# USNavalResearchLaboratory/mgen

Hardware: AMD Instinct MI355X
Metric: device-resident MgenMsg pack+unpack GB/s and Mmsg/s at 1/2/4/8 MI355X (higher is better)
Workload: dtype u8; 1 GPU; udp_unpack_crc_1M_x_1024B; records_per_gpu=1048576, record_bytes=1024, checksum=True, output=mgenx_rec rows (32 B), parallelism=flow-sharded x1 (independent slabs)

## Files before the change

### mgen_amd/csrc/mgenx_api.hip

```cpp
#include <hipcub/hipcub.hpp>
#include <hsa/hsa.h>
#include <hsa/hsa_ext_amd.h>
#include <immintrin.h>

#include <math.h>
#include <stdio.h>
#include <string.h>

#include <algorithm>
#include <chrono>
#include <emmintrin.h>
#include <atomic>
#include <mutex>
#include <vector>


#include "mgenx_kernels.hpp"
#include "mgenx_flowdist.hpp"
#if MGENX_DIAG
#include "mgenx_diag.h"
#endif

extern "C" void* mgenx_scan_ws_new();
extern "C" void mgenx_scan_ws_free(void* p);
// ... 353 lines not shown
  for (mgenx_worker* w : c->workers) worker_detach(w);
  c->workers.clear();
  void* ps[] = {c->d_tabs, c->d_expect, c->d_xpow, c->d_ia, c->d_bytetab, c->d_rtab, c->d_rcrc,
                c->d_sink, c->d_rq};
  if (c->scan_ws) mgenx_scan_ws_free(c->scan_ws);
  if (c->flow_ws) mgenx_flow_ws_free(c->flow_ws);
  if (c->flowdist_ws) mgenx_flowdist_ws_free(c->flowdist_ws);
  if (c->log_ws) mgenx_log_ws_free(c->log_ws);
  mgenx::dev_free(c->tcp_ws);
  mgenx::dev_free(c->tcp_plan);
  mgenx::dev_free(c->rx_ws);
  mgenx::host_free(c->tcp_host);
  for (mgenx_grow& g : c->bl) g.release();
  c->snap.release();
  c->defrag.release();
  c->lp.release();
  for (void* p : ps) mgenx::dev_free(p);
  delete c;
  return MGENX_OK;
}

int mgenx_unpack_batch(mgenx_ctx* ctx, const uint8_t* dev_slab, uint64_t slab_bytes,
                       const uint64_t* dev_rec_off, uint64_t stride,
                       const uint32_t* dev_rec_len, uint32_t fixed_len, uint32_t n,
                       const mgenx_cols* cols, uint32_t opts, void* stream) {
  if (!ctx || !cols) return MGENX_EINVAL;
  if (n == 0) return MGENX_OK;
  if (!dev_slab) return MGENX_EINVAL;
  if (!dev_rec_off && stride == 0 && n > 1) return MGENX_EINVAL;
  const mgenx_cols& k = *cols;
  if (!k.rows && (!k.flow_id || !k.seq_num || !k.tx_sec || !k.tx_usec || !k.msg_len ||
                  !k.dst_port || !k.flags || !k.err || !k.dst_type || !k.dst_len ||
                  !k.dst_addr4 || !k.payload_len || !k.payload_type || !k.gps_status))
    return MGENX_EINVAL;
  mgenx::UnpackParams p;
  p.slab = dev_slab;
  p.slab_bytes = slab_bytes;
  p.rec_off = dev_rec_off;
  p.stride = stride;
  p.rec_len = dev_rec_len;
  p.fixed_len = fixed_len;
  p.n = n;
  p.opts = opts;
  p.tabs = ctx->d_tabs;
  p.expect = ctx->d_expect;
  p.expect_fixed = fixed_len < ctx->h_expect.size() ? ctx->h_expect[fixed_len] : 0u;
  p.sink = ctx->d_sink;
  p.variant = MGENX_DIAG ? ctx->unpack_variant : 0;
  p.cols = k;
  const uint64_t groups = ((uint64_t)n + 15) / 16;
  const uint64_t per_block = (uint64_t)mgenx::unpack_threads() / 64;
  uint64_t grid = (groups + per_block - 1) / per_block;
  if (grid > (uint64_t)ctx->cu_count) grid = ctx->cu_count;
  hipError_t e = mgenx::launch_unpack(p, (int)grid, (hipStream_t)stream, &ctx->unpack_last);
  return e == hipSuccess ? MGENX_OK : set_err(ctx, e, "unpack");
}

int mgenx_unpack_last_kernel(const mgenx_ctx* ctx) { return ctx ? ctx->unpack_last : 0; }

int mgenx_pack_prepare(mgenx_ctx* ctx, const mgenx_flow_tmpl* dev_tmpl, uint32_t n_tmpl,
                       const uint8_t* dev_pool, uint32_t* dev_tmpl_crc, void* stream) {
  if (!ctx || (n_tmpl && (!dev_tmpl || !dev_tmpl_crc))) return MGENX_EINVAL;
  hipError_t e = mgenx::launch_pack_prepare(dev_tmpl, n_tmpl, dev_pool, ctx->d_bytetab,
                                            dev_tmpl_crc, (hipStream_t)stream);
  return e == hipSuccess ? MGENX_OK : set_err(ctx, e, "pack_prepare");
}

int mgenx_set_fill_time(mgenx_ctx* ctx, uint32_t fill_time) {
  if (!ctx) return MGENX_EINVAL;
  if (ctx->rand_ready && ctx->rand_time == fill_time) return MGENX_OK;
  std::vector<uint8_t> rt(16 + kN + 32, 0);
  glibc_rand_bytes(fill_time, kN, &rt[16]);
  uint32_t t[256];
  byte_table(t);
  std::vector<uint32_t> rc(kN);
  uint32_t c = 0;
  for (uint32_t k = 0; k < kN; k++) {
    rc[k] = c;
    c = t[(c ^ rt[16 + k]) & 0xffu] ^ (c >> 8);
  }
  hipSetDevice(ctx->device);
  hipError_t e = hipMemcpy(ctx->d_rtab, rt.data(), rt.size(), hipMemcpyHostToDevice);
  if (e == hipSuccess) e = hipMemcpy(ctx->d_rcrc, rc.data(), kN * 4, hipMemcpyHostToDevice);
  if (e != hipSuccess) return set_err(ctx, e, "set_fill_time");
  ctx->rand_ready = true;
  ctx->rand_time = fill_time;
  return MGENX_OK;
}

static int pack_common(mgenx_ctx* ctx, const mgenx_flow_tmpl* dev_tmpl,
                       const uint32_t* dev_tmpl_crc, const mgenx_pack_desc* dev_desc, uint32_t n,
                       const uint8_t* dev_pool, uint8_t* dev_slab, uint64_t slab_bytes,
                       const uint64_t* dev_rec_off, uint64_t stride, const uint32_t* dev_buf_len,
                       const uint32_t* dev_crc_in, uint32_t* dev_out_len, uint32_t* dev_tx_crc,
                       uint32_t* dev_state, uint32_t opts, uint32_t fill_time, void* stream,
                       const uint32_t* dev_frag_len = nullptr, int frag_ck = 0,
                       const uint32_t* dev_skip = nullptr) {
  if (!ctx) return MGENX_EINVAL;
  if (n == 0) return MGENX_OK;
  if (!dev_tmpl || !dev_tmpl_crc || !dev_desc || !dev_slab || !dev_out_len) return MGENX_EINVAL;
  if (!dev_rec_off && stride == 0 && n > 1) return MGENX_EINVAL;
  if (opts & MGENX_PACK_RANDOM_FILL) {
    if (!ctx->rand_ready || ctx->rand_time != fill_time) return MGENX_EINVAL;
  }
  mgenx::PackParams p;
  p.tmpl = dev_tmpl;
  p.tmpl_crc = dev_tmpl_crc;
// ... 1296 lines not shown
```

### mgen_amd/csrc/mgenx_kernels.hpp

```cpp
#pragma once

#include "mgenx_common.hpp"

#include <mutex>
#include <set>
#include <utility>

#ifndef MGENX_DIAG
#define MGENX_DIAG 0
#endif

namespace mgenx {

void quiesce_workers(int device);
inline void dev_free(void* p) {
  if (!p) return;
  int dev = -1;
  if (hipGetDevice(&dev) != hipSuccess) dev = -1;
  quiesce_workers(dev);
  (void)hipFree(p);
}
inline void host_free(void* p) {
  if (!p) return;
  quiesce_workers(-1);
// ... 8 lines not shown
  static std::set<std::pair<const void*, int>> done;
  std::lock_guard<std::mutex> g(mu);
  if (done.count({fn, dev})) return hipSuccess;
  e = hipFuncSetAttribute(fn, hipFuncAttributeMaxDynamicSharedMemorySize, bytes);
  if (e == hipSuccess) done.insert({fn, dev});
  return e;
}

struct UnpackParams {
  const uint8_t* slab;
  uint64_t slab_bytes;
  const uint64_t* rec_off;
  uint64_t stride;
  const uint32_t* rec_len;
  uint32_t fixed_len;
  uint32_t n;
  uint32_t opts;
  const uint32_t* tabs;
  const uint32_t* expect;
  uint32_t expect_fixed;
  uint8_t* sink;
  int variant;
  mgenx_cols cols;
};

struct PackParams {
  const mgenx_flow_tmpl* tmpl;
  const uint32_t* tmpl_crc;
  const mgenx_pack_desc* desc;
  uint32_t n;
  const uint8_t* pool;
  uint8_t* slab;
  uint64_t slab_bytes;
  const uint64_t* rec_off;
  uint64_t stride;
  uint32_t* out_len;
  uint32_t opts;
  const uint32_t* byte_tab;
  const uint32_t* a4_tab;
  const uint32_t* xpow;
  const uint32_t* ia;
  const uint8_t* rtab;
  const uint32_t* rcrc;
  const uint32_t* buf_len;
  const uint32_t* crc_in;
  uint32_t* tx_crc;
  uint32_t* state;
  const uint32_t* frag_len;
  int frag_ck;
  int variant;
  const uint32_t* skip = nullptr;
};

hipError_t launch_unpack(const UnpackParams& p, int grid, hipStream_t stream, int* which);
int unpack_threads();
#if MGENX_DIAG
hipError_t launch_group_rw(const uint8_t* p, uint64_t bytes, uint8_t* out, int mode, int grid,
                           hipStream_t stream);
hipError_t launch_stream_read(const uint8_t* p, uint64_t bytes, uint32_t* out, int grid,
                              hipStream_t stream);
hipError_t launch_stream_read_w(const uint8_t* p, uint64_t bytes, uint32_t* out, int grid,
                                int width, hipStream_t stream);
#endif
hipError_t launch_pack(const PackParams& p, int grid, hipStream_t stream);
hipError_t launch_pack_prepare(const mgenx_flow_tmpl* tmpl, uint32_t n_tmpl, const uint8_t* pool,
                               const uint32_t* byte_tab, uint32_t* out, hipStream_t stream);
constexpr int kRqUnqTime = 0;
constexpr int kRqThrTime = 256;
constexpr int kRqLog10Lo = -40;
constexpr int kRqLog10N = 65;
constexpr int kRqThrLog10 = 512;
constexpr int kRqP10 = 512 + 65;
constexpr int kRqP10N = 309;
constexpr int kRqDoubles = 512 + 65 + 309;

hipError_t launch_rx_persist(const mgenx_cols& c, uint32_t n, uint32_t opts, int32_t* ws,
                             mgenx_rx_state* state, const uint8_t* slab, const uint64_t* rec_off,
                             const uint32_t* rec_len, const uint32_t* byte_tab,
                             uint32_t* payload_rec, hipStream_t s);
size_t rx_persist_ws_bytes(uint32_t n);
hipError_t launch_tcp_plan(const mgenx_flow_tmpl* tmpl, const mgenx_pack_desc* desc,
                           const uint32_t* msg_total, uint32_t n, uint64_t* bytes,
                           uint32_t* nfrag, uint32_t* max_frag, hipStream_t s);
hipError_t launch_tcp_frag(const mgenx_pack_desc* desc, const uint32_t* msg_total,
                           const uint32_t* nfrag, const uint64_t* msg_off, uint32_t n, uint32_t r,
                           int ck, const uint32_t* prev_state, mgenx_pack_desc* fd, uint64_t* foff,
                           uint32_t* fbuf, uint32_t* ff, hipStream_t s);
constexpr uint32_t kTcpPlanMsgs = 1024;
constexpr uint32_t kTcpPlanEpochs = 1u << 16;
hipError_t launch_tcp_plan0(const mgenx_flow_tmpl* tmpl, const mgenx_pack_desc* desc,
                            const uint32_t* msg_total, uint32_t n, int ck, uint64_t cap,
                            uint32_t epoch, uint64_t* status, uint64_t* fmax, uint64_t* msg_off,
                            uint32_t* nfrag, mgenx_pack_desc* fd, uint32_t* fbuf, uint32_t* ff,
                            uint32_t* skip, uint64_t* host, hipStream_t s);
constexpr uint32_t kWorkUnpack = 1, kWorkCrc32 = 2, kWorkPack = 3, kWorkRecv = 4, kWorkUpdate = 5,
                   kWorkStop = 15;
constexpr uint32_t kWorkerMaxBytes = MGENX_WORKER_MAX_BYTES;
constexpr uint32_t kWorkerHdrBytes = 1024;
constexpr uint32_t kWorkerPackMax = MGENX_WORKER_PACK_MAX;
struct WPackReq {
  mgenx_flow_tmpl tmpl;
  mgenx_pack_desc desc;
  uint32_t buf_len, crc_in, opts, rsv;
};
struct WUpdReq {
  uint64_t flows;
  uint32_t slot, seq, rx_sec, rx_usec, tx_sec, tx_usec, msg, rsv;
// ... 30 lines not shown
```

### mgen_amd/csrc/mgenx_unpack.hip

```cpp
#include <type_traits>

#include "mgenx_kernels.hpp"
#include "mgenx_parse.hpp"

namespace mgenx {

constexpr int kUnpackThreads = 1024;
constexpr int kRep = 32;
constexpr int kRepDwords = 4 * 256 * kRep;
constexpr int kSmallTabDwords = 1024;
constexpr int kFoldTabs = 6;
constexpr size_t kUnpackLdsBytes = (size_t)(kRepDwords + kFoldTabs * kSmallTabDwords) * 4u;


__device__ __forceinline__ uint32_t a64_s1(uint32_t lane) { return ((lane & 31u) << 2) | (1u << 16); }

typedef __attribute__((address_space(3))) uint32_t lds_u32_t;
__device__ __forceinline__ uint32_t lds_u32(const uint8_t*, uint32_t addr, uint32_t imm) {
  return *(const lds_u32_t*)(addr + imm);
}

__device__ __forceinline__ uint32_t xor3(uint32_t a, uint32_t b, uint32_t c) {
  return __builtin_amdgcn_bitop3_b32(a, b, c, 0x96);
}

__device__ __forceinline__ void a64_parts(const uint8_t* ldsb, uint32_t c, uint32_t s1,
                                          uint32_t& ha, uint32_t& hb) {
  const uint32_t t0 = lds_u32(ldsb, __builtin_amdgcn_perm(c, s1, 0x0c0c0400u), 0);
  const uint32_t t1 = lds_u32(ldsb, __builtin_amdgcn_perm(c, s1, 0x0c0c0500u), 128);
  const uint32_t t2 = lds_u32(ldsb, __builtin_amdgcn_perm(c, s1, 0x0c020600u), 0);
  const uint32_t t3 = lds_u32(ldsb, __builtin_amdgcn_perm(c, s1, 0x0c020700u), 128);
  ha = xor3(t0, t1, t2);
  hb = t3;
}

struct TableRegs {
  uint32_t a64, fold[kFoldTabs];
};
__device__ __forceinline__ TableRegs table_loads(const uint32_t* tabs) {
  TableRegs r;
  r.a64 = tabs[threadIdx.x];
#pragma unroll
  for (int k = 0; k < kFoldTabs; k++) r.fold[k] = tabs[1024 + k * 1024 + threadIdx.x];
  return r;
}
__device__ __forceinline__ void table_writes(uint32_t* lds, const TableRegs& r) {
  typedef __attribute__((address_space(3))) u32x4_t lds_u32x4_t;
  const uint32_t e = threadIdx.x;
  const uint32_t k = e >> 8, val = e & 255u;
  const u32x4_t s = {r.a64, r.a64, r.a64, r.a64};
  lds_u32x4_t* dst = (lds_u32x4_t*)((k >> 1) * 65536u + val * 256u + (k & 1u) * 128u);
#pragma unroll
  for (int c = 0; c < kRep / 4; c++) dst[c] = s;
  uint32_t* fold = lds + kRepDwords;
#pragma unroll
  for (int k2 = 0; k2 < kFoldTabs; k2++) fold[k2 * 1024 + e] = r.fold[k2];
}
__device__ __forceinline__ void stage_tables(uint32_t* lds, const uint32_t* tabs) {
  table_writes(lds, table_loads(tabs));
}

__device__ __forceinline__ uint32_t shift_tab(const uint32_t* t, uint32_t x) {
  return t[x & 0xffu] ^ t[256 + ((x >> 8) & 0xffu)] ^ t[512 + ((x >> 16) & 0xffu)] ^
         t[768 + (x >> 24)];
}

__device__ __forceinline__ u32x4_t shl_bytes(u32x4_t v, int s) {
  const int a = s >> 2;
  const int c = (s & 3) * 8;
  uint32_t w[4] = {v.x, v.y, v.z, v.w};
  uint32_t o[4];
#pragma unroll
  for (int i = 0; i < 4; i++) {
    const int hi_i = i - a, lo_i = i - a - 1;
    uint32_t hi = 0, lo = 0;
#pragma unroll
    for (int k = 0; k < 4; k++) {
      hi = (k == hi_i) ? w[k] : hi;
      lo = (k == lo_i) ? w[k] : lo;
    }
    o[i] = c ? ((hi << c) | (lo >> (32 - c))) : hi;
  }
  return u32x4_t{o[0], o[1], o[2], o[3]};
}


__device__ __forceinline__ bool fast_layout(uint32_t w0, uint32_t w5, uint32_t hw) {
  const uint32_t t = (w5 >> 16) & 0xffu;
  const uint32_t D = w5 >> 24;
  const uint32_t H = hw >> 24;
  return ((w0 >> 16) & 0xffu) == 2u && (t == 1u || t == 2u) && (D == 4u || D == 16u) &&
         (H == 0u || H == 4u || H == 16u) && D + H <= 20u;
}

__device__ bool small_crc_ok(const uint8_t* r, uint32_t L) {
  if (L < 4) return false;
  uint32_t c = 0xFFFFFFFFu;
  for (uint32_t i = 0; i < L - 4; i++) {
    c ^= r[i];
#pragma unroll
    for (int k = 0; k < 8; k++) c = (c >> 1) ^ ((c & 1u) ? kPoly : 0u);
  }
  c ^= 0xFFFFFFFFu;
  const uint32_t t = ((uint32_t)r[L - 4] << 24) | ((uint32_t)r[L - 3] << 16) |
                     ((uint32_t)r[L - 2] << 8) | r[L - 1];
  return c == t;
}

__device__ __forceinline__ uint32_t prefix_word(const u32x4_t& pf, int k) {
// ... 773 lines not shown
        } else {
#pragma unroll
          for (int j = 0; j < 8; j++) w[j] = 0;
        }
        const bool flagged = force || (((w[0] >> 24) & MGENX_FLAG_CHECKSUM) != 0 &&
                                       buf_len >= MGENX_MIN_SIZE && ((w[0] >> 16) & 0xffu) == 2u);
        const bool needs_crc = flagged && (tcp ? (G.L >= 4) : fixed_ok(buf_len, w));
        const bool vec_crc = needs_crc && G.L >= 32;
        Hdr h;
        parse_header(rec, buf_len, want_ext, w, h);
        const bool crc_ok = !needs_crc || (vec_crc ? (tot == expect) : small_crc_ok(rec, G.L));
        store_hdr_q0(p.cols, G.idx, h, crc_ok, tcp);
      } else if (G.oob && q == 0) {
        store_oob_q0(p.cols, G.idx);
      }
    }

    if (KB > 0 && burst && held == (uint32_t)KH) flush();
    if (!has_next) break;
    pf = ldu128(hdr_ptr(N));
    expect = p.expect[N.live ? N.L : 0u];
    if (next_tile) {
      t_c = t_p;
      t_p = t_c + n_waves;
      off_c = off_p;
      len_c = len_p;
      src_c = src_p;
      place(t_p, off_p, len_p);
      p_ranked = false;
      k = 0;
    } else {
      k++;
    }
    G = N;
  }
  if (KB > 0 && burst && held) flush();
}

template <int NR, int MODE = 0, bool kRows = false, bool kAligned = false>
__global__ void __launch_bounds__(kUnpackThreads)
unpack_fixed_kernel(UnpackParams p, uint32_t expect) {
  constexpr bool kAblXor = (MODE & 1) != 0, kAblNoTail = (MODE & 2) != 0;
  constexpr bool kAblNoStore = (MODE & 4) != 0, kAblSink = (MODE & 8) != 0;
  constexpr bool kAblAltStore = (MODE & 16) != 0;
  constexpr bool kAblWrap = (MODE & 32) != 0;
  constexpr bool kAblWt = (MODE & 64) != 0;
  constexpr bool kAblNtLoad = (MODE & 128) != 0;
  constexpr bool kAblBurst = (MODE & 256) != 0;
  constexpr bool kAblBurstSeq = (MODE & 512) != 0;
  extern __shared__ __attribute__((aligned(16))) uint32_t lds[];
  uint32_t* rep = lds;
  uint32_t* fold = lds + kRepDwords;
  const uint8_t* ldsb = reinterpret_cast<const uint8_t*>(rep);
  const TableRegs tab_regs = table_loads(p.tabs);
  asm volatile("" ::: "memory");

  const int lane = threadIdx.x & 63;
  const int q = lane & 3;
  const uint32_t s1 = a64_s1((uint32_t)lane);
  const uint32_t wave_id = __builtin_amdgcn_readfirstlane(
      blockIdx.x * (blockDim.x >> 6) + (threadIdx.x >> 6));
  const uint32_t n_waves = gridDim.x * (blockDim.x >> 6);
  const uint32_t n_groups = (p.n + 15u) >> 4;
  const bool force = (p.opts & MGENX_OPT_CHECKSUM_FORCE) != 0;
  const bool tcp = (p.opts & MGENX_OPT_TCP) != 0;
  const uint32_t L = p.fixed_len;
  constexpr int V = NR;

  uint32_t g = wave_id;
  const uint32_t g_end = n_groups;

  auto rec_idx = [&](uint32_t gg) { return (gg << 4) + (uint32_t)(lane >> 2); };
  auto rec_ptr = [&](uint32_t i) { return p.slab + (uint64_t)i * p.stride; };
  auto is_live = [&](uint32_t i) {
    const uint64_t off = (uint64_t)i * p.stride;
    return i < p.n && off <= p.slab_bytes && L <= p.slab_bytes - off;
  };
  auto base_off = [&](bool lv, uint32_t i) { return lv ? i * (uint32_t)p.stride : 64u; };
  const int pos0 = (int)L - 64 * V + 16 * q;
  auto ld = [&](uint32_t off, int imm) {
    if (kAblNtLoad) return ldnt128(p.slab + (uint64_t)off + imm);
    return ldu128(p.slab + (uint64_t)off + imm);
  };
  auto ld_row = [&](uint32_t boff, int j) {
    return j == 0 ? ld(boff + (uint32_t)(pos0 > 0 ? pos0 : 0), 0)
                  : ld(boff + (uint32_t)(pos0 + 64), 64 * (j - 1));
  };
  auto ld_hdr = [&](uint32_t boff) { return ld(boff + 16u * (uint32_t)q, 0); };

  u32x4_t d[NR];
  struct Out {
    uint32_t o[5];
  };
  auto decode = [&](const u32x4_t& pf, uint32_t idx, bool live) {
    uint32_t w[8];
#pragma unroll
    for (int j = 0; j < 8; j++) w[j] = prefix_word(pf, j);
    const uint32_t w10 = prefix_word(pf, 10);
    const uint32_t D = w[5] >> 24;
    const uint32_t hw = (D == 4u) ? w[7] : w10;
    const uint32_t gi = (28u + D + (hw >> 24)) >> 2;
    const uint32_t g3 = (prefix_word(pf, 11) & (0u - (uint32_t)(gi == 8u))) |
                        (prefix_word(pf, 12) & (0u - (uint32_t)(gi == 9u))) |
                        (prefix_word(pf, 14) & (0u - (uint32_t)(gi == 11u))) |
                        (prefix_word(pf, 15) & (0u - (uint32_t)(gi == 12u)));
    uint32_t flow = bswap32(w[1]), seq = bswap32(w[2]), sec = bswap32(w[3]);
    uint32_t usec = bswap32(w[4]), dst4 = w[6];
// ... 190 lines not shown
      __builtin_amdgcn_sched_barrier(0);
      const uint32_t v = shift_tab(fold + 3 * 1024, f0) ^ shift_tab(fold + 2 * 1024, f1) ^
                         shift_tab(fold + 1 * 1024, f2) ^ shift_tab(fold, f3);
      const uint32_t* lt = fold + (q == 0 ? 5 : (q == 1 ? 4 : 3)) * 1024;
      uint32_t s = (q == 3) ? v : shift_tab(lt, v);
      s ^= __shfl_xor(s, 1);
      s ^= __shfl_xor(s, 2);
      if (kAblNoTail) {
        if (s == 0x9E3779B9u && lane == 0) p.cols.err[idx] = (uint8_t)needs_crc;
      } else {
        const Out r = kAligned ? early : decode(hdr, idx, live);
        emit(r, idx, needs_crc && s != expect);
      }
      asm volatile("" ::"v"(boff_n + (uint32_t)(pos0 + 64)));
      g = gn;
      idx = idx_n;
      live = live_n;
      return has_next && any;
    };
    u32x4_t pf2;
    if (kAligned) {
      while (step(pf, pf2)) {
      }
    } else {
      for (;;) {
        if (!step(pf, pf2)) break;
        if (!step(pf2, pf)) break;
      }
    }
    for (; g < g_end; g += n_waves) {
      const uint32_t i = rec_idx(g);
      const bool lv = is_live(i);
      const u32x4_t ph = ld_hdr(base_off(lv, i));
      const bool nc = decide(ph, lv);
      if (__any(nc)) break;
      emit(decode(ph, i, lv), i, false);
    }
  }
  if (kAblBurst) {
    uint32_t k = 0;
    for (uint32_t gg = wave_id; gg < g_end; gg += n_waves, k++) {
      const uint32_t i = rec_idx(gg);
      const uint64_t seq = (uint64_t)wave_id * 8192u + k * 512u + 8u * (uint32_t)lane;
      const uint64_t a = (uint64_t)p.cols.rows + (kAblBurstSeq ? seq : (uint64_t)i * 32 + 8 * q);
      if (i < p.n) {
        if (kAblWt) st_g64_wt(a, (uint64_t)gg);
        else if (kAblAltStore) st_g64(a, (uint64_t)gg);
        else st_g64_nt(a, (uint64_t)gg);
      }
    }
  }
}

template <int NR, int RS = 4, int K = 16>
__global__ void __launch_bounds__(kUnpackThreads)
unpack_fixed_ring_kernel(UnpackParams p, uint32_t expect) {
  static_assert(NR == 8 || NR == 16, "ring kernel: 512- or 1024-byte records");
  static_assert(NR % RS == 0, "the ring divides the record's rows");
  extern __shared__ __attribute__((aligned(16))) uint32_t lds[];
  const uint32_t* fold = lds + kRepDwords;
  const uint8_t* ldsb = reinterpret_cast<const uint8_t*>(lds);
  const TableRegs tab_regs = table_loads(p.tabs);
  asm volatile("" ::: "memory");

  const int lane = threadIdx.x & 63;
  const int q = lane & 3;
  const uint32_t s1 = a64_s1((uint32_t)lane);
  const uint32_t wave_id = __builtin_amdgcn_readfirstlane(
      blockIdx.x * (blockDim.x >> 6) + (threadIdx.x >> 6));
  const uint32_t n_waves = gridDim.x * (blockDim.x >> 6);
  const uint32_t g_end = (p.n + 15u) >> 4;
  const bool force = (p.opts & MGENX_OPT_CHECKSUM_FORCE) != 0;
  const bool tcp = (p.opts & MGENX_OPT_TCP) != 0;
  const uint32_t L = p.fixed_len;

  auto rec_idx = [&](uint32_t gg) { return (gg << 4) + (uint32_t)(lane >> 2); };
  auto is_live = [&](uint32_t i) {
    const uint64_t off = (uint64_t)i * p.stride;
    return (bool)((i < p.n) & (off <= p.slab_bytes) & (L <= p.slab_bytes - off));
  };
  auto row_base = [&](uint32_t i, bool live) {
    return (live ? i * (uint32_t)p.stride : 64u) + 16u * (uint32_t)q;
  };
  const uint32_t qm0 = 0u - (uint32_t)(q == 0), qm1 = 0u - (uint32_t)(q == 1);
  const uint32_t qm2 = 0u - (uint32_t)(q == 2), qm3 = 0u - (uint32_t)(q == 3);
  auto ld = [&](uint32_t base, int j) { return ldu128(p.slab + (uint64_t)base + 64 * j); };
  auto decide = [&](const u32x4_t& pf, bool live) {
    const uint32_t w0 = prefix_word(pf, 0);
    const uint32_t w5 = prefix_word(pf, 5);
    const bool v2 = ((w0 >> 16) & 0xffu) == 2u;
    const bool flagged = force || ((((w0 >> 24) & MGENX_FLAG_CHECKSUM) != 0) && v2);
    const uint32_t t = (w5 >> 16) & 0xffu;
    return live && flagged && (tcp || (v2 && (t == 1u || t == 2u)));
  };
  auto decode = [&](const u32x4_t& pf, uint32_t idx, bool live, uint32_t& o0, uint32_t& o1) {
    uint32_t w[8];
#pragma unroll
    for (int j = 0; j < 8; j++) w[j] = prefix_word(pf, j);
    const uint32_t w10 = prefix_word(pf, 10);
    const uint32_t D = w[5] >> 24;
    const uint32_t hw = (D == 4u) ? w[7] : w10;
    const uint32_t gi = (28u + D + (hw >> 24)) >> 2;
    const uint32_t g3 = (prefix_word(pf, 11) & (0u - (uint32_t)(gi == 8u))) |
                        (prefix_word(pf, 12) & (0u - (uint32_t)(gi == 9u))) |
                        (prefix_word(pf, 14) & (0u - (uint32_t)(gi == 11u))) |
                        (prefix_word(pf, 15) & (0u - (uint32_t)(gi == 12u)));
    uint32_t flow = bswap32(w[1]), seq = bswap32(w[2]), sec = bswap32(w[3]);
    uint32_t usec = bswap32(w[4]), dst4 = w[6];
    uint32_t msg_len = bswap16((uint16_t)(w[0] & 0xffffu));
    uint32_t dport = bswap16((uint16_t)(w[5] & 0xffffu));
    const uint32_t hlen = 44u + D + (hw >> 24);
    uint32_t plen = bswap16((uint16_t)(g3 >> 16));
    if (!(plen != 0 && hlen + plen <= L)) plen = 0;
    uint32_t flags = w[0] >> 24, err = 0, dtype = (w[5] >> 16) & 0xffu, dlen = D;
    uint32_t ptype = (g3 >> 8) & 0xffu, gps = g3 & 0xffu;
    const bool slow = live && !fast_layout(w[0], w[5], hw);
    if (__any(slow)) {
      Hdr h;
      if (slow && q == 0) parse_header(p.slab + (uint64_t)idx * p.stride, L, false, w, h);
      auto bc = [&](uint32_t& dst, uint32_t v) {
        v = (uint32_t)__builtin_amdgcn_mov_dpp((int)v, 0x00, 0xf, 0xf, false);
        if (slow) dst = v;
      };
      bc(flow, h.flow); bc(seq, h.seq); bc(sec, h.sec); bc(usec, h.usec); bc(dst4, h.dst4);
      bc(msg_len, h.msg_len); bc(dport, h.dst_port); bc(plen, h.plen); bc(flags, h.flags);
      bc(err, h.err); bc(dtype, h.dst_type); bc(dlen, h.dst_len); bc(ptype, h.ptype);
      bc(gps, h.gps);
    }
    const uint32_t a3 = plen | flags << 16 | err << 24;
    const uint32_t c3 = dtype | dlen << 8 | ptype << 16 | gps << 24;
    const uint32_t c2 = msg_len | dport << 16;
    const uint32_t r0 = (flow & qm0) | (sec & qm1) | (dst4 & qm2) | (a3 & qm3);
    const uint32_t r1 = (seq & qm0) | (usec & qm1) | (c2 & qm2) | (c3 & qm3);
    o0 = live ? r0 : (qm3 & ((uint32_t)MGENX_ERROR_OOB << 24));
    o1 = live ? r1 : 0u;
  };
  auto verdict = [&](uint32_t& o0, bool crc_bad) {
    const uint32_t fl = tcp ? (uint32_t)MGENX_FLAG_CHECKSUM_ERROR : 0u;
    if (crc_bad && q == 3) o0 = (o0 & 0x00ffffffu) | fl << 16 | (uint32_t)MGENX_ERROR_CHECKSUM << 24;
  };

  typedef uint32_t held_t __attribute__((ext_vector_type(K)));
  held_t b0 = 0u, b1 = 0u;
  uint32_t held = 0, last_g = 0;
  uint32_t left = __builtin_amdgcn_readfirstlane(
      wave_id < g_end ? (g_end - 1u - wave_id) / n_waves + 1u : 0u);
  uint32_t slot = (uint32_t)K - (left < (uint32_t)K ? left : (uint32_t)K);
  auto push = [&](uint32_t o0, uint32_t o1, uint32_t gg) {
    const uint32_t us = __builtin_amdgcn_readfirstlane(slot);
    b0[us] = o0;
    b1[us] = o1;
    slot++;
    held++;
    left--;
    last_g = gg;
  };
  auto flush = [&]() {
#pragma unroll
    for (int k = 0; k < K; k++) {
      const uint32_t back = (uint32_t)(K - 1 - k);
      const uint32_t gg = last_g - back * n_waves;
      const uint32_t idx = rec_idx(gg);
      const bool in = back < held && idx < p.n;
      const uint64_t v = (uint64_t)b1[k] << 32 | b0[k];
      if (back < held)
        st_g64_nt(in ? (uint64_t)p.cols.rows + (uint64_t)idx * 32 + 8 * q
                     : (uint64_t)p.sink + 8u * (uint32_t)lane, v);
    }
    held = 0;
    slot = (uint32_t)K - (left < (uint32_t)K ? left : (uint32_t)K);
  };

  u32x4_t d[RS];
  uint32_t g = wave_id;
  uint32_t idx = rec_idx(g < g_end ? g : 0u);
  bool live = is_live(idx);
  uint32_t base = row_base(idx, live);
#pragma unroll
  for (int j = 0; j < RS; j++) {
    d[j] = ld(base, j);
    __builtin_amdgcn_sched_barrier(0);
  }
  table_writes(lds, tab_regs);
  asm volatile("s_waitcnt lgkmcnt(0)" ::: "memory");
  __builtin_amdgcn_s_barrier();
  if (g >= g_end) return;

  for (;;) {
    bool more;
    do {
      const uint32_t gn = g + n_waves;
      const bool has_next = gn < g_end;
      const uint32_t idx_n = rec_idx(has_next ? gn : g);
      const bool live_n = is_live(idx_n);
      const uint32_t base_n = row_base(idx_n, live_n);
      const u32x4_t hdr = d[0];
      const bool needs_crc = decide(hdr, live);
      const bool any = __any(needs_crc);
      uint32_t o0, o1;
      decode(hdr, idx, live, o0, o1);
      uint32_t ha[4] = {0u, 0u, 0u, 0u}, hb[4] = {0u, 0u, 0u, 0u};
#pragma unroll
      for (int j = 0; j < NR - 1; j++) {
        const u32x4_t x = d[j % RS];
        const uint32_t xw[4] = {x.x, x.y, x.z, x.w};
        uint32_t c4[4];
#pragma unroll
        for (int b = 0; b < 4; b++) c4[b] = xor3(ha[b], hb[b], xw[b]);
        __builtin_amdgcn_sched_barrier(0);
        if ((j % RS) == RS - 1) {
#pragma unroll
          for (int t = j - (RS - 1); t <= j; t++)
            d[t % RS] = (t + RS < NR) ? ld(base, t + RS) : ld(base_n, t + RS - NR);
        }
        __builtin_amdgcn_sched_barrier(0);
#pragma unroll
        for (int b = 0; b < 4; b++) a64_parts(ldsb, c4[b], s1, ha[b], hb[b]);
      }
      const u32x4_t xf = d[(NR - 1) % RS];
      uint32_t f0 = xor3(ha[0], hb[0], xf.x), f1 = xor3(ha[1], hb[1], xf.y);
      uint32_t f2 = xor3(ha[2], hb[2], xf.z);
      uint32_t f3 = xor3(ha[3], hb[3], q == 3 ? bswap32(xf.w) : xf.w);
      asm volatile("" : "+v"(f0), "+v"(f1), "+v"(f2), "+v"(f3));
      __builtin_amdgcn_sched_barrier(0);
#pragma unroll
      for (int t = NR - RS; t < NR; t++) d[t % RS] = ld(base_n, t + RS - NR);
      __builtin_amdgcn_sched_barrier(0);
      const uint32_t v = shift_tab(fold + 3 * 1024, f0) ^ shift_tab(fold + 2 * 1024, f1) ^
                         shift_tab(fold + 1 * 1024, f2) ^ shift_tab(fold, f3);
      const uint32_t* lt = fold + (q == 0 ? 5 : (q == 1 ? 4 : 3)) * 1024;
      uint32_t sum = (q == 3) ? v : shift_tab(lt, v);
      sum ^= __shfl_xor(sum, 1);
      sum ^= __shfl_xor(sum, 2);
      verdict(o0, needs_crc && sum != expect);
      push(o0, o1, g);
      if (held == (uint32_t)K) flush();
      g = gn;
      idx = idx_n;
      live = live_n;
      base = base_n;
      more = has_next && any;
    } while (more);
    for (; g < g_end; g += n_waves) {
      idx = rec_idx(g);
      live = is_live(idx);
      base = row_base(idx, live);
      const u32x4_t ph = ld(base, 0);
      if (__any(decide(ph, live))) break;
      uint32_t o0, o1;
      decode(ph, idx, live, o0, o1);
      push(o0, o1, g);
      if (held == (uint32_t)K) flush();
    }
    if (g >= g_end) break;
    for (int j = 0; j < RS; j++) d[j] = ld(base, j);
  }
  if (held) flush();
}

constexpr int kLongNB = 8;
constexpr uint32_t kLongMin = 4096;
constexpr int kLongFold = 7;
constexpr size_t kLongLdsBytes = (size_t)(kRepDwords + kLongFold * kSmallTabDwords) * 4u;
static_assert(kLongLdsBytes <= 160u * 1024u, "long-record tables fit the CU's LDS");

template <int NB = kLongNB, int NT = kUnpackThreads>
__global__ void __launch_bounds__(NT) unpack_long_kernel(UnpackParams p) {
  static_assert(1024 % NT == 0, "table staging: whole passes");
  extern __shared__ __attribute__((aligned(16))) uint32_t lds[];
  const uint32_t* fold = lds + kRepDwords;
  const uint32_t *fA4 = fold, *fA16 = fold + 1024, *fA32 = fold + 2048, *fA64 = fold + 3072,
                 *fA128 = fold + 4096, *fA256 = fold + 5120, *fA512 = fold + 6144;
  const uint8_t* ldsb = reinterpret_cast<const uint8_t*>(lds);
  constexpr int kFoldIdx[kLongFold] = {kTabA4, kTabA16, kTabA32, kTabA64, kTabA128, kTabA256,
                                       kTabA512};
  const uint32_t a1024 = p.tabs[kTabA1024 * 1024 + threadIdx.x];
  uint32_t fr[kLongFold];
#pragma unroll
  for (int k = 0; k < kLongFold; k++) fr[k] = p.tabs[kFoldIdx[k] * 1024 + threadIdx.x];
  constexpr int kNB = NB;

  const int lane = threadIdx.x & 63;
  const int q = lane & 3, quad = lane >> 2;
  const uint32_t s1 = a64_s1((uint32_t)lane);
  const uint32_t wave_id = __builtin_amdgcn_readfirstlane(
      blockIdx.x * (blockDim.x >> 6) + (threadIdx.x >> 6));
  const uint32_t n_waves = gridDim.x * (blockDim.x >> 6);
  const bool force = (p.opts & MGENX_OPT_CHECKSUM_FORCE) != 0;
  const bool tcp = (p.opts & MGENX_OPT_TCP) != 0;
  const bool want_ext = p.cols.dst_addr || p.cols.host_addr;
  const mgenx_cols& cc = p.cols;
  const bool any_ext = cc.hdr_len || cc.payload_off || cc.host_port || cc.host_type ||
                       cc.host_len || cc.lat_raw || cc.lon_raw || cc.alt || cc.dst_addr ||
                       cc.host_addr || cc.decoded;
  const uint8_t* dummy = reinterpret_cast<const uint8_t*>(p.tabs);

  struct Rec {
    uint32_t idx;
    uint64_t off;
    uint32_t L;
    bool live;
    bool rows;
    uint32_t nb;
    int64_t r0;
  };
  auto place = [&](uint32_t ri) {
    Rec r;
    r.idx = ri;
// ... 172 lines not shown
}

template <int MODE>
static hipError_t launch_mode(const UnpackParams& p, int grid, hipStream_t stream) {
  return launch_lds(unpack_kernel<true, MODE>, p, grid, stream);
}

template <int NT = kUnpackThreads, int KB = 4, int MODE = 0>
static hipError_t launch_var(const UnpackParams& p, int grid, hipStream_t stream) {
  hipError_t e = set_max_lds((const void*)unpack_var_kernel<NT, KB, MODE>, (int)kUnpackLdsBytes);
  if (e != hipSuccess) return e;
  hipLaunchKernelGGL((unpack_var_kernel<NT, KB, MODE>), dim3(grid), dim3(NT), kUnpackLdsBytes,
                     stream, p);
  return hipGetLastError();
}

template <int NB = kLongNB, int NT = kUnpackThreads>
static hipError_t launch_long_t(const UnpackParams& p, int grid, hipStream_t stream) {
  hipError_t e = set_max_lds((const void*)unpack_long_kernel<NB, NT>, (int)kLongLdsBytes);
  if (e != hipSuccess) return e;
  hipLaunchKernelGGL((unpack_long_kernel<NB, NT>), dim3(grid), dim3(NT), kLongLdsBytes, stream, p);
  return hipGetLastError();
}
static hipError_t launch_long(const UnpackParams& p, int grid, hipStream_t stream) {
#if MGENX_DIAG
  switch (p.variant) {
    case 40: return launch_long_t<16, 512>(p, grid, stream);
    case 41: return launch_long_t<8, 512>(p, grid, stream);
    case 42: return launch_long_t<4, 1024>(p, grid, stream);
    case 43: return launch_long_t<12, 512>(p, grid, stream);
    case 44: return launch_long_t<2, 1024>(p, grid, stream);
    case 45: return launch_long_t<16, 1024>(p, grid, stream);
    default: break;
  }
#endif
  return launch_long_t<>(p, grid, stream);
}

#if MGENX_DIAG
static hipError_t launch_sorted(const UnpackParams& p, int grid, hipStream_t stream) {
  return launch_lds(unpack_kernel<true, 0, true>, p, grid, stream);
}
#endif

template <int NR, int MODE = 0, bool kRows = false, bool kAligned = false>
static hipError_t launch_fixed(const UnpackParams& p, int grid, hipStream_t stream) {
  hipError_t e = set_max_lds((const void*)unpack_fixed_kernel<NR, MODE, kRows, kAligned>, (int)kUnpackLdsBytes);
  if (e != hipSuccess) return e;
  hipLaunchKernelGGL((unpack_fixed_kernel<NR, MODE, kRows, kAligned>), dim3(grid),
                     dim3(kUnpackThreads), kUnpackLdsBytes, stream, p, p.expect_fixed);
  return hipGetLastError();
}

template <int NR, int RS = 4, int K = 16>
static hipError_t launch_ring(const UnpackParams& p, int grid, hipStream_t stream) {
  hipError_t e = set_max_lds((const void*)unpack_fixed_ring_kernel<NR, RS, K>, (int)kUnpackLdsBytes);
  if (e != hipSuccess) return e;
  hipLaunchKernelGGL((unpack_fixed_ring_kernel<NR, RS, K>), dim3(grid), dim3(kUnpackThreads),
                     kUnpackLdsBytes, stream, p, p.expect_fixed);
  return hipGetLastError();
}

typedef hipError_t (*fixed_launcher)(const UnpackParams&, int, hipStream_t);
#define MGENX_FIXED_TABLE(R)                                                              \
  {nullptr, nullptr, launch_fixed<2, 0, R>, launch_fixed<3, 0, R>, launch_fixed<4, 0, R>,    \
   launch_fixed<5, 0, R>, launch_fixed<6, 0, R>, launch_fixed<7, 0, R>, launch_fixed<8, 0, R>, \
   launch_fixed<9, 0, R>, launch_fixed<10, 0, R>, launch_fixed<11, 0, R>,                    \
   launch_fixed<12, 0, R>, launch_fixed<13, 0, R>, launch_fixed<14, 0, R>,                   \
   launch_fixed<15, 0, R>, launch_fixed<16, 0, R>}
static const fixed_launcher kFixedLaunch[17] = MGENX_FIXED_TABLE(false);
static const fixed_launcher kFixedLaunchRows[17] = MGENX_FIXED_TABLE(true);
#undef MGENX_FIXED_TABLE

hipError_t launch_unpack(const UnpackParams& p, int grid, hipStream_t stream, int* which) {
  const int unpack_variant = p.variant;
  *which = MGENX_UNPACK_K_OTHER;
  if (p.opts & MGENX_OPT_SKIP_CRC) {
    *which = MGENX_UNPACK_K_HEADER;
    hipLaunchKernelGGL((unpack_kernel<false>), dim3(grid), dim3(kUnpackThreads), 0, stream, p);
    return hipGetLastError();
  }
  const mgenx_cols& c = p.cols;
  const bool ext = c.hdr_len || c.payload_off || c.host_port || c.host_type || c.host_len ||
                   c.lat_raw || c.lon_raw || c.alt || c.dst_addr || c.host_addr || c.decoded;
  const uint32_t nr = (p.fixed_len + 63) / 64;
  const bool fixed = !p.rec_off && !p.rec_len && p.fixed_len >= 65 && p.fixed_len <= 1024 &&
                     p.stride > 0 && p.n <= 0xFFFFFFF0u && !ext &&
                     p.slab_bytes < 0xFFFF0000ull && p.slab_bytes >= 64ull * (nr + 1) + 16 &&
                     p.slab_bytes >= p.fixed_len;
  if (unpack_variant == 0 && fixed) {
    *which = (c.rows && (p.fixed_len == 512 || p.fixed_len == 1024)) ? MGENX_UNPACK_K_FIXED_RING
                                                                    : MGENX_UNPACK_K_FIXED;
    switch (p.fixed_len) {
      case 256: return c.rows ? launch_fixed<4, 0, true, true>(p, grid, stream)
                              : launch_fixed<4, 0, false, true>(p, grid, stream);
      case 512: return c.rows ? launch_ring<8>(p, grid, stream)
                              : launch_fixed<8, 0, false, true>(p, grid, stream);
      case 1024: return c.rows ? launch_ring<16>(p, grid, stream)
                               : launch_fixed<16, 0, false, true>(p, grid, stream);
      default: break;
    }
    return (c.rows ? kFixedLaunchRows : kFixedLaunch)[(p.fixed_len + 63) / 64](p, grid, stream);
  }
#if MGENX_DIAG
  if (unpack_variant == 13 && fixed && p.fixed_len == 1024)
    return c.rows ? launch_fixed<16, 0, true, true>(p, grid, stream)
                  : launch_fixed<16, 0, false, true>(p, grid, stream);
  if (unpack_variant >= 14 && unpack_variant <= 16 && fixed && p.fixed_len == 1024 && c.rows) {
    if (unpack_variant == 14) return launch_ring<16, 8, 12>(p, grid, stream);
    if (unpack_variant == 15) return launch_ring<16, 8, 8>(p, grid, stream);
    return launch_ring<16, 4, 12>(p, grid, stream);
  }
  if (unpack_variant == 12 && fixed && p.fixed_len == 1024)
    return c.rows ? launch_fixed<16, 0, true>(p, grid, stream) : launch_fixed<16, 0>(p, grid, stream);
  if (unpack_variant >= 1024 && fixed && p.fixed_len == 1024) {
    switch (unpack_variant - 1024) {
#define MGENX_ABL(M) \
  case M: return c.rows ? launch_fixed<16, M, true, true>(p, grid, stream) \
                        : launch_fixed<16, M, false, true>(p, grid, stream);
      MGENX_ABL(1) MGENX_ABL(2) MGENX_ABL(3) MGENX_ABL(4) MGENX_ABL(5) MGENX_ABL(8)
      MGENX_ABL(16) MGENX_ABL(32) MGENX_ABL(64)
      MGENX_ABL(128) MGENX_ABL(144) MGENX_ABL(130) MGENX_ABL(136) MGENX_ABL(260) MGENX_ABL(772)
      MGENX_ABL(276) MGENX_ABL(324) MGENX_ABL(788)
#undef MGENX_ABL
      default: break;
    }
  }
  switch (unpack_variant) {
    case 1: return launch_mode<1>(p, grid, stream);
    case 2: return launch_mode<2>(p, grid, stream);
    case 3: return launch_mode<0>(p, grid, stream);
    case 4: return launch_sorted(p, grid, stream);
    default: break;
  }
  if (p.rec_len && unpack_variant >= 20 && unpack_variant < 40) {
    *which = MGENX_UNPACK_K_VAR;
    switch (unpack_variant) {
      case 20: return launch_var<1024, 0, 1>(p, grid, stream);
      case 21: return launch_var<1024, 0, 0>(p, grid, stream);
      case 22: return launch_var<768, 8, 0>(p, grid, stream);
      case 23: return launch_var<768, 16, 0>(p, grid, stream);
      case 27: return launch_var<1024, 8, 0>(p, grid, stream);
      case 32: return launch_var<1024, 4, 8>(p, grid, stream);
      case 33: return launch_var<1024, 4, 16>(p, grid, stream);
      default: break;
    }
  }
#endif
  const uint64_t mean = p.rec_len ? (p.n ? p.slab_bytes / p.n : 0) : p.fixed_len;
  if (mean >= kLongMin) {
    *which = MGENX_UNPACK_K_LONG;
    return launch_long(p, grid, stream);
  }
  const uint64_t tiles = ((uint64_t)p.n + 63) / 64;
  const uint64_t waves = (uint64_t)grid * (kUnpackThreads / 64);
  if (p.rec_len && tiles >= 2 * waves) {
    *which = MGENX_UNPACK_K_VAR;
    return launch_var(p, grid, stream);
  }
  *which = MGENX_UNPACK_K_GENERAL;
  return launch_mode<0>(p, grid, stream);
}

#if MGENX_DIAG
// ... 239 lines not shown
```

Before: 5962 GB/s.

## Generalize unpack ring kernel with multi-record prefetch and non-temporal slab loads

The fixed-length ring unpack kernel is templated on block rows, number of blocks, wave count and a non-temporal-load flag. The ring can now prefetch rows from more than one record ahead, and table staging is split across fewer threads. By default the 1024-byte rows path switches to non-temporal loads for the streamed slab, and the 512-byte path does so only when the batch is large. The aim is to keep the streamed slab from polluting cache so load bandwidth improves, at the cost of added template complexity and many diagnostic variants.

```diff
diff --git a/mgen_amd/csrc/mgenx_api.hip b/mgen_amd/csrc/mgenx_api.hip
--- a/mgen_amd/csrc/mgenx_api.hip
+++ b/mgen_amd/csrc/mgenx_api.hip
@@ -429,7 +429,8 @@
   const uint64_t per_block = (uint64_t)mgenx::unpack_threads() / 64;
   uint64_t grid = (groups + per_block - 1) / per_block;
   if (grid > (uint64_t)ctx->cu_count) grid = ctx->cu_count;
-  hipError_t e = mgenx::launch_unpack(p, (int)grid, (hipStream_t)stream, &ctx->unpack_last);
+  hipError_t e = mgenx::launch_unpack(p, (int)grid, ctx->cu_count, (hipStream_t)stream,
+                                      &ctx->unpack_last);
   return e == hipSuccess ? MGENX_OK : set_err(ctx, e, "unpack");
 }
 
diff --git a/mgen_amd/csrc/mgenx_kernels.hpp b/mgen_amd/csrc/mgenx_kernels.hpp
--- a/mgen_amd/csrc/mgenx_kernels.hpp
+++ b/mgen_amd/csrc/mgenx_kernels.hpp
@@ -84,7 +84,8 @@
   const uint32_t* skip = nullptr;
 };
 
-hipError_t launch_unpack(const UnpackParams& p, int grid, hipStream_t stream, int* which);
+hipError_t launch_unpack(const UnpackParams& p, int grid, int cus, hipStream_t stream,
+                         int* which);
 int unpack_threads();
 #if MGENX_DIAG
 hipError_t launch_group_rw(const uint8_t* p, uint64_t bytes, uint8_t* out, int mode, int grid,
diff --git a/mgen_amd/csrc/mgenx_unpack.hip b/mgen_amd/csrc/mgenx_unpack.hip
--- a/mgen_amd/csrc/mgenx_unpack.hip
+++ b/mgen_amd/csrc/mgenx_unpack.hip
@@ -34,27 +34,39 @@
   hb = t3;
 }
 
+template <int NT = 1024>
 struct TableRegs {
-  uint32_t a64, fold[kFoldTabs];
+  static_assert(1024 % NT == 0, "every thread stages the same number of entries");
+  static constexpr int kPer = 1024 / NT;
+  uint32_t a64[kPer], fold[kFoldTabs][kPer];
 };
-__device__ __forceinline__ TableRegs table_loads(const uint32_t* tabs) {
-  TableRegs r;
-  r.a64 = tabs[threadIdx.x];
-#pragma unroll
-  for (int k = 0; k < kFoldTabs; k++) r.fold[k] = tabs[1024 + k * 1024 + threadIdx.x];
+template <int NT = 1024>
+__device__ __forceinline__ TableRegs<NT> table_loads(const uint32_t* tabs) {
+  TableRegs<NT> r;
+#pragma unroll
+  for (int i = 0; i < r.kPer; i++) {
+    const uint32_t e = threadIdx.x + (uint32_t)(i * NT);
+    r.a64[i] = tabs[e];
+#pragma unroll
+    for (int k = 0; k < kFoldTabs; k++) r.fold[k][i] = tabs[1024 + k * 1024 + e];
+  }
   return r;
 }
-__device__ __forceinline__ void table_writes(uint32_t* lds, const TableRegs& r) {
+template <int NT>
+__device__ __forceinline__ void table_writes(uint32_t* lds, const TableRegs<NT>& r) {
   typedef __attribute__((address_space(3))) u32x4_t lds_u32x4_t;
-  const uint32_t e = threadIdx.x;
-  const uint32_t k = e >> 8, val = e & 255u;
-  const u32x4_t s = {r.a64, r.a64, r.a64, r.a64};
-  lds_u32x4_t* dst = (lds_u32x4_t*)((k >> 1) * 65536u + val * 256u + (k & 1u) * 128u);
-#pragma unroll
-  for (int c = 0; c < kRep / 4; c++) dst[c] = s;
   uint32_t* fold = lds + kRepDwords;
 #pragma unroll
-  for (int k2 = 0; k2 < kFoldTabs; k2++) fold[k2 * 1024 + e] = r.fold[k2];
+  for (int i = 0; i < r.kPer; i++) {
+    const uint32_t e = threadIdx.x + (uint32_t)(i * NT);
+    const uint32_t k = e >> 8, val = e & 255u;
+    const u32x4_t s = {r.a64[i], r.a64[i], r.a64[i], r.a64[i]};
+    lds_u32x4_t* dst = (lds_u32x4_t*)((k >> 1) * 65536u + val * 256u + (k & 1u) * 128u);
+#pragma unroll
+    for (int c = 0; c < kRep / 4; c++) dst[c] = s;
+#pragma unroll
+    for (int k2 = 0; k2 < kFoldTabs; k2++) fold[k2 * 1024 + e] = r.fold[k2][i];
+  }
 }
 __device__ __forceinline__ void stage_tables(uint32_t* lds, const uint32_t* tabs) {
   table_writes(lds, table_loads(tabs));
@@ -934,7 +946,7 @@
   uint32_t* rep = lds;
   uint32_t* fold = lds + kRepDwords;
   const uint8_t* ldsb = reinterpret_cast<const uint8_t*>(rep);
-  const TableRegs tab_regs = table_loads(p.tabs);
+  const TableRegs<> tab_regs = table_loads(p.tabs);
   asm volatile("" ::: "memory");
 
   const int lane = threadIdx.x & 63;
@@ -1231,15 +1243,18 @@
   }
 }
 
-template <int NR, int RS = 4, int K = 16>
-__global__ void __launch_bounds__(kUnpackThreads)
+template <int NR, int BR = 4, int NB = 1, int K = 16, int NW = 16, bool kNt = false>
+__global__ void __launch_bounds__(NW * 64)
 unpack_fixed_ring_kernel(UnpackParams p, uint32_t expect) {
+  constexpr int RS = NB * BR;
+  constexpr int G = RS > NR ? RS / NR : 1;
   static_assert(NR == 8 || NR == 16, "ring kernel: 512- or 1024-byte records");
-  static_assert(NR % RS == 0, "the ring divides the record's rows");
+  static_assert(NR % BR == 0, "a block lies inside one record");
+  static_assert(RS <= NR ? NR % RS == 0 : (RS == 2 * NR && BR == NR), "static ring indices");
   extern __shared__ __attribute__((aligned(16))) uint32_t lds[];
   const uint32_t* fold = lds + kRepDwords;
   const uint8_t* ldsb = reinterpret_cast<const uint8_t*>(lds);
-  const TableRegs tab_regs = table_loads(p.tabs);
+  const TableRegs<NW * 64> tab_regs = table_loads<NW * 64>(p.tabs);
   asm volatile("" ::: "memory");
 
   const int lane = threadIdx.x & 63;
@@ -1263,7 +1278,10 @@
   };
   const uint32_t qm0 = 0u - (uint32_t)(q == 0), qm1 = 0u - (uint32_t)(q == 1);
   const uint32_t qm2 = 0u - (uint32_t)(q == 2), qm3 = 0u - (uint32_t)(q == 3);
-  auto ld = [&](uint32_t base, int j) { return ldu128(p.slab + (uint64_t)base + 64 * j); };
+  auto ld = [&](uint32_t base, int j) {
+    const uint8_t* a = p.slab + (uint64_t)base + 64 * j;
+    return kNt ? ldnt128(a) : ldu128(a);
+  };
   auto decide = [&](const u32x4_t& pf, bool live) {
     const uint32_t w0 = prefix_word(pf, 0);
     const uint32_t w5 = prefix_word(pf, 5);
@@ -1352,59 +1370,80 @@
 
   u32x4_t d[RS];
   uint32_t g = wave_id;
-  uint32_t idx = rec_idx(g < g_end ? g : 0u);
-  bool live = is_live(idx);
-  uint32_t base = row_base(idx, live);
-#pragma unroll
-  for (int j = 0; j < RS; j++) {
-    d[j] = ld(base, j);
-    __builtin_amdgcn_sched_barrier(0);
-  }
+  uint32_t idxq[G];
+  bool liveq[G];
+  uint32_t base = 0;
+  auto prime = [&]() {
+    const uint32_t g0 = g < g_end ? g : 0u;
+#pragma unroll
+    for (int s = 0; s < G; s++) {
+      const uint32_t gs = g + (uint32_t)s * n_waves;
+      idxq[s] = rec_idx(gs < g_end ? gs : g0);
+      liveq[s] = is_live(idxq[s]);
+      const uint32_t b = row_base(idxq[s], liveq[s]);
+      if (s == 0) base = b;
+#pragma unroll
+      for (int j = 0; j < (RS < NR ? RS : NR); j++) {
+        d[s * NR + j] = ld(b, j);
+        __builtin_amdgcn_sched_barrier(0);
+      }
+    }
+  };
+  prime();
   table_writes(lds, tab_regs);
   asm volatile("s_waitcnt lgkmcnt(0)" ::: "memory");
   __builtin_amdgcn_s_barrier();
   if (g >= g_end) return;
 
-  for (;;) {
-    bool more;
-    do {
-      const uint32_t gn = g + n_waves;
-      const bool has_next = gn < g_end;
-      const uint32_t idx_n = rec_idx(has_next ? gn : g);
-      const bool live_n = is_live(idx_n);
-      const uint32_t base_n = row_base(idx_n, live_n);
-      const u32x4_t hdr = d[0];
-      const bool needs_crc = decide(hdr, live);
-      const bool any = __any(needs_crc);
-      uint32_t o0, o1;
+  auto step = [&](auto slot_c, bool run) -> bool {
+    constexpr int S = decltype(slot_c)::value;
+    constexpr auto ri = [](int j) { return (S * NR + j) % RS; };
+    const uint32_t idx = idxq[0];
+    const bool live = liveq[0];
+    const bool has_next = g + n_waves < g_end;
+    const uint32_t gn = g + (uint32_t)G * n_waves;
+    const uint32_t idx_n = rec_idx(gn < g_end ? gn : g);
+    const bool live_n = is_live(idx_n);
+    const uint32_t base_n = row_base(idx_n, live_n);
+    bool needs_crc = false, any = false;
+    uint32_t o0 = 0u, o1 = 0u, f0 = 0u, f1 = 0u, f2 = 0u, f3 = 0u;
+    if (run) {
+      const u32x4_t hdr = d[ri(0)];
+      needs_crc = decide(hdr, live);
+      any = __any(needs_crc);
       decode(hdr, idx, live, o0, o1);
       uint32_t ha[4] = {0u, 0u, 0u, 0u}, hb[4] = {0u, 0u, 0u, 0u};
 #pragma unroll
       for (int j = 0; j < NR - 1; j++) {
-        const u32x4_t x = d[j % RS];
+        const u32x4_t x = d[ri(j)];
         const uint32_t xw[4] = {x.x, x.y, x.z, x.w};
         uint32_t c4[4];
 #pragma unroll
         for (int b = 0; b < 4; b++) c4[b] = xor3(ha[b], hb[b], xw[b]);
         __builtin_amdgcn_sched_barrier(0);
-        if ((j % RS) == RS - 1) {
-#pragma unroll
-          for (int t = j - (RS - 1); t <= j; t++)
-            d[t % RS] = (t + RS < NR) ? ld(base, t + RS) : ld(base_n, t + RS - NR);
+        if ((j % BR) == BR - 1) {
+#pragma unroll
+          for (int t = j - (BR - 1); t <= j; t++) {
+            if (t + RS < NR) d[ri(t)] = ldu128(p.slab + (uint64_t)base + 64 * (t + RS));
+            else d[ri(t)] = ld(base_n, (t + RS) % NR);
+          }
         }
         __builtin_amdgcn_sched_barrier(0);
 #pragma unroll
         for (int b = 0; b < 4; b++) a64_parts(ldsb, c4[b], s1, ha[b], hb[b]);
       }
-      const u32x4_t xf = d[(NR - 1) % RS];
-      uint32_t f0 = xor3(ha[0], hb[0], xf.x), f1 = xor3(ha[1], hb[1], xf.y);
-      uint32_t f2 = xor3(ha[2], hb[2], xf.z);
-      uint32_t f3 = xor3(ha[3], hb[3], q == 3 ? bswap32(xf.w) : xf.w);
-      asm volatile("" : "+v"(f0), "+v"(f1), "+v"(f2), "+v"(f3));
-      __builtin_amdgcn_sched_barrier(0);
-#pragma unroll
-      for (int t = NR - RS; t < NR; t++) d[t % RS] = ld(base_n, t + RS - NR);
-      __builtin_amdgcn_sched_barrier(0);
+      const u32x4_t xf = d[ri(NR - 1)];
+      f0 = xor3(ha[0], hb[0], xf.x);
+      f1 = xor3(ha[1], hb[1], xf.y);
+      f2 = xor3(ha[2], hb[2], xf.z);
+      f3 = xor3(ha[3], hb[3], q == 3 ? bswap32(xf.w) : xf.w);
+    }
+    asm volatile("" : "+v"(f0), "+v"(f1), "+v"(f2), "+v"(f3));
+    __builtin_amdgcn_sched_barrier(0);
+#pragma unroll
+    for (int t = NR - BR; t < NR; t++) d[ri(t)] = ld(base_n, (t + RS) % NR);
+    __builtin_amdgcn_sched_barrier(0);
+    if (run) {
       const uint32_t v = shift_tab(fold + 3 * 1024, f0) ^ shift_tab(fold + 2 * 1024, f1) ^
                          shift_tab(fold + 1 * 1024, f2) ^ shift_tab(fold, f3);
       const uint32_t* lt = fold + (q == 0 ? 5 : (q == 1 ? 4 : 3)) * 1024;
@@ -1414,25 +1453,42 @@
       verdict(o0, needs_crc && sum != expect);
       push(o0, o1, g);
       if (held == (uint32_t)K) flush();
-      g = gn;
-      idx = idx_n;
-      live = live_n;
-      base = base_n;
-      more = has_next && any;
-    } while (more);
+      g += n_waves;
+#pragma unroll
+      for (int s = 0; s + 1 < G; s++) {
+        idxq[s] = idxq[s + 1];
+        liveq[s] = liveq[s + 1];
+      }
+      idxq[G - 1] = idx_n;
+      liveq[G - 1] = live_n;
+      if (G == 1) base = base_n;
+    }
+    return run && has_next && any;
+  };
+
+  for (;;) {
+    if (G == 1) {
+      while (step(std::integral_constant<int, 0>{}, true)) {
+      }
+    } else {
+      bool more;
+      do {
+        const bool two = step(std::integral_constant<int, 0>{}, true);
+        more = step(std::integral_constant<int, G - 1>{}, two);
+      } while (more);
+    }
     for (; g < g_end; g += n_waves) {
-      idx = rec_idx(g);
-      live = is_live(idx);
-      base = row_base(idx, live);
-      const u32x4_t ph = ld(base, 0);
-      if (__any(decide(ph, live))) break;
+      const uint32_t i = rec_idx(g);
+      const bool lv = is_live(i);
+      const u32x4_t ph = ldu128(p.slab + (uint64_t)row_base(i, lv));
+      if (__any(decide(ph, lv))) break;
       uint32_t o0, o1;
-      decode(ph, idx, live, o0, o1);
+      decode(ph, i, lv, o0, o1);
       push(o0, o1, g);
       if (held == (uint32_t)K) flush();
     }
     if (g >= g_end) break;
-    for (int j = 0; j < RS; j++) d[j] = ld(base, j);
+    prime();
   }
   if (held) flush();
 }
@@ -1711,14 +1767,20 @@
   return hipGetLastError();
 }
 
-template <int NR, int RS = 4, int K = 16>
-static hipError_t launch_ring(const UnpackParams& p, int grid, hipStream_t stream) {
-  hipError_t e = set_max_lds((const void*)unpack_fixed_ring_kernel<NR, RS, K>, (int)kUnpackLdsBytes);
+template <int NR, int BR = 4, int NB = 1, int K = 16, int NW = 16, bool kNt = false>
+static hipError_t launch_ring(const UnpackParams& p, int cus, hipStream_t stream) {
+  const auto kernel = unpack_fixed_ring_kernel<NR, BR, NB, K, NW, kNt>;
+  hipError_t e = set_max_lds((const void*)kernel, (int)kUnpackLdsBytes);
   if (e != hipSuccess) return e;
-  hipLaunchKernelGGL((unpack_fixed_ring_kernel<NR, RS, K>), dim3(grid), dim3(kUnpackThreads),
-                     kUnpackLdsBytes, stream, p, p.expect_fixed);
+  const uint64_t groups = ((uint64_t)p.n + 15) / 16;
+  uint64_t grid = (groups + NW - 1) / NW;
+  if (grid > (uint64_t)cus) grid = (uint64_t)cus;
+  hipLaunchKernelGGL(kernel, dim3((unsigned)grid), dim3(NW * 64), kUnpackLdsBytes, stream, p,
+                     p.expect_fixed);
   return hipGetLastError();
 }
+
+constexpr uint32_t kRingNt512Groups = 24576;
 
 typedef hipError_t (*fixed_launcher)(const UnpackParams&, int, hipStream_t);
 #define MGENX_FIXED_TABLE(R)                                                              \
@@ -1731,7 +1793,8 @@
 static const fixed_launcher kFixedLaunchRows[17] = MGENX_FIXED_TABLE(true);
 #undef MGENX_FIXED_TABLE
 
-hipError_t launch_unpack(const UnpackParams& p, int grid, hipStream_t stream, int* which) {
+hipError_t launch_unpack(const UnpackParams& p, int grid, int cus, hipStream_t stream,
+                         int* which) {
   const int unpack_variant = p.variant;
   *which = MGENX_UNPACK_K_OTHER;
   if (p.opts & MGENX_OPT_SKIP_CRC) {
@@ -1753,9 +1816,12 @@
     switch (p.fixed_len) {
       case 256: return c.rows ? launch_fixed<4, 0, true, true>(p, grid, stream)
                               : launch_fixed<4, 0, false, true>(p, grid, stream);
-      case 512: return c.rows ? launch_ring<8>(p, grid, stream)
-                              : launch_fixed<8, 0, false, true>(p, grid, stream);
-      case 1024: return c.rows ? launch_ring<16>(p, grid, stream)
+      case 512:
+        if (!c.rows) return launch_fixed<8, 0, false, true>(p, grid, stream);
+        return (p.n + 15u) / 16u >= kRingNt512Groups
+                   ? launch_ring<8, 4, 1, 16, 16, true>(p, cus, stream)
+                   : launch_ring<8, 4, 1, 16, 16, false>(p, cus, stream);
+      case 1024: return c.rows ? launch_ring<16, 4, 1, 16, 16, true>(p, cus, stream)
                                : launch_fixed<16, 0, false, true>(p, grid, stream);
       default: break;
     }
@@ -1766,9 +1832,68 @@
     return c.rows ? launch_fixed<16, 0, true, true>(p, grid, stream)
                   : launch_fixed<16, 0, false, true>(p, grid, stream);
   if (unpack_variant >= 14 && unpack_variant <= 16 && fixed && p.fixed_len == 1024 && c.rows) {
-    if (unpack_variant == 14) return launch_ring<16, 8, 12>(p, grid, stream);
-    if (unpack_variant == 15) return launch_ring<16, 8, 8>(p, grid, stream);
-    return launch_ring<16, 4, 12>(p, grid, stream);
+    if (unpack_variant == 14) return launch_ring<16, 8, 1, 12>(p, cus, stream);
+    if (unpack_variant == 15) return launch_ring<16, 8, 1, 8>(p, cus, stream);
+    return launch_ring<16, 4, 1, 12>(p, cus, stream);
+  }
+  if (unpack_variant >= 17 && unpack_variant <= 19 && fixed && c.rows &&
+      (p.fixed_len == 1024 || (p.fixed_len == 512 && unpack_variant != 19))) {
+    *which = MGENX_UNPACK_K_FIXED_RING;
+    const bool r16 = p.fixed_len == 1024;
+    if (unpack_variant == 17)
+      return r16 ? launch_ring<16, 4, 1, 16, 16>(p, cus, stream)
+                 : launch_ring<8, 4, 1, 16, 16>(p, cus, stream);
+    if (unpack_variant == 18)
+      return r16 ? launch_ring<16, 8, 2, 32, 8>(p, cus, stream)
+                 : launch_ring<8, 8, 2, 32, 8>(p, cus, stream);
+    return launch_ring<16, 4, 4, 32, 8>(p, cus, stream);
+  }
+  if (unpack_variant >= 20 && unpack_variant <= 22 && fixed && c.rows && !p.rec_len &&
+      (p.fixed_len == 512 || p.fixed_len == 1024)) {
+    *which = MGENX_UNPACK_K_FIXED_RING;
+    const bool r16 = p.fixed_len == 1024;
+    if (unpack_variant == 20)
+      return r16 ? launch_ring<16, 4, 2, 16, 16>(p, cus, stream)
+                 : launch_ring<8, 4, 2, 16, 16>(p, cus, stream);
+    if (unpack_variant == 21)
+      return r16 ? launch_ring<16, 2, 4, 16, 16>(p, cus, stream)
+                 : launch_ring<8, 2, 4, 16, 16>(p, cus, stream);
+    return r16 ? launch_ring<16, 2, 2, 16, 16>(p, cus, stream)
+               : launch_ring<8, 2, 2, 16, 16>(p, cus, stream);
+  }
+  if (unpack_variant >= 27 && unpack_variant <= 32 && fixed && c.rows && !p.rec_len &&
+      (p.fixed_len == 512 || p.fixed_len == 1024)) {
+    *which = MGENX_UNPACK_K_FIXED_RING;
+    const bool r16 = p.fixed_len == 1024;
+    switch (unpack_variant) {
+      case 27: return r16 ? launch_ring<16, 8, 2, 32, 8, true>(p, cus, stream)
+                          : launch_ring<8, 8, 2, 32, 8, true>(p, cus, stream);
+      case 28: return r16 ? launch_ring<16, 4, 1, 16, 16, true>(p, cus, stream)
+                          : launch_ring<8, 4, 1, 16, 16, true>(p, cus, stream);
+      case 29: return r16 ? launch_ring<16, 4, 2, 16, 16, true>(p, cus, stream)
+                          : launch_ring<8, 4, 2, 16, 16, true>(p, cus, stream);
+      case 30: return r16 ? launch_ring<16, 2, 1, 16, 16, true>(p, cus, stream)
+                          : launch_ring<8, 2, 1, 16, 16, true>(p, cus, stream);
+      case 31: return r16 ? launch_ring<16, 8, 1, 32, 8, true>(p, cus, stream)
+                          : launch_ring<8, 8, 1, 32, 8, true>(p, cus, stream);
+      default: return r16 ? launch_ring<16, 8, 1, 16, 16, true>(p, cus, stream)
+                          : launch_ring<8, 8, 1, 16, 16, true>(p, cus, stream);
+    }
+  }
+  if (unpack_variant >= 23 && unpack_variant <= 26 && fixed && c.rows && !p.rec_len &&
+      (p.fixed_len == 1024 || (p.fixed_len == 512 && unpack_variant != 26))) {
+    *which = MGENX_UNPACK_K_FIXED_RING;
+    const bool r16 = p.fixed_len == 1024;
+    if (unpack_variant == 23)
+      return r16 ? launch_ring<16, 8, 1, 16, 16>(p, cus, stream)
+                 : launch_ring<8, 8, 1, 16, 16>(p, cus, stream);
+    if (unpack_variant == 24)
+      return r16 ? launch_ring<16, 2, 1, 16, 16>(p, cus, stream)
+                 : launch_ring<8, 2, 1, 16, 16>(p, cus, stream);
+    if (unpack_variant == 25)
+      return r16 ? launch_ring<16, 8, 1, 32, 8>(p, cus, stream)
+                 : launch_ring<8, 8, 1, 32, 8>(p, cus, stream);
+    return launch_ring<16, 16, 1, 32, 8>(p, cus, stream);
   }
   if (unpack_variant == 12 && fixed && p.fixed_len == 1024)
     return c.rows ? launch_fixed<16, 0, true>(p, grid, stream) : launch_fixed<16, 0>(p, grid, stream);
```

Result: faster. 6411 GB/s (median of 6 runs) (+7.5%).
